# Distributed-Deep-Learning/ErasureHead

Hardware: AMD Instinct MI355X
Metric: wall-clock sec/iter + iters-to-loss-floor, logistic regression n_stragglers=2, 1/2/4/8 MI355X (lower is better)
Workload: dtype fp64

## Files before the change

### csrc/bindings.cpp

```cpp
#include <c10/hip/HIPStream.h>
#include <pybind11/stl.h>
#include <torch/extension.h>

#include <optional>
#include <stdexcept>
#include <string>
#include <tuple>
#include <vector>

#include "runtime/collector.h"

#include "kernels/grad_dense.h"
#include "kernels/launchers.h"

extern "C" const char eh_source_hash[];

namespace eh {
void bind_ipc(pybind11::module& m);
void bind_comm(pybind11::module& m);
void bind_engine(pybind11::module& m);
}

namespace {

// ... 29 lines not shown
       "part must hold [nslots*16*ld] partial sums (acc dtype)");
}

void grad_dense(int64_t dtype, int64_t loss, int64_t cpl, const Tensor& segs, const Tensor& tasks,
                const Tensor& beta, const Tensor& slab, const Tensor& slot_task_begin, const Tensor& part,
                const Tensor& G, int64_t ld, const eh::KernelChoice& choice) {
  need_cuda(segs, "segs");
  need_cuda(tasks, "tasks");
  need_cuda(beta, "beta");
  need_cuda(slab, "slab");
  need_cuda(slot_task_begin, "slot_task_begin");
  need_cuda(G, "G");
  const int64_t ntasks = tasks.size(0);
  const int64_t nslots = slot_task_begin.numel() - 1;
  need(tasks.dim() == 2 && tasks.size(1) == 5 && tasks.scalar_type() == at::kInt, "tasks must be int32 [ntasks, 5]");
  need(segs.scalar_type() == at::kByte && segs.numel() % 32 == 0, "segs must be packed uint8 [nseg*32]");
  need(slab.dim() == 2 && slab.size(0) >= ntasks && slab.size(1) == ld, "slab must be [>=ntasks, ld]");
  need(G.dim() == 2 && G.size(0) == nslots && G.size(1) == ld, "G must be [nslots, ld]");
  need(beta.numel() >= ld, "beta must have >= ld elements");
  need(ld % (dtype == 0 ? 2 : dtype == 1 ? 4 : 8) == 0, "ld must be a multiple of the 16-byte vector width");
  need(cpl <= 32 ? cpl * 64 >= ld
                   : ((cpl == 256 || cpl == 512) && cpl * (dtype == 0 ? 16 : 32) >= ld),
         "cpl (narrow: columns per lane, wide: block size) must cover ld");
  const int ac = dtype == 0 ? 0 : 1;
  need(acc_code(beta) == ac && acc_code(slab) == ac && acc_code(G) == ac, "beta/slab/G dtype mismatch");
  need_part(part, nslots, ld, ac);
  if (ntasks == 0) return;
  check(eh::grad_dense_launch((int)dtype, (int)loss, (int)cpl, segs.data_ptr(), tasks.data_ptr(), (int)ntasks,
                              beta.data_ptr(), slab.data_ptr(), slot_task_begin.data_ptr<int>(), (int)nslots,
                              part.data_ptr(), G.data_ptr(), (int)ld, stream_of(G), choice),
        "grad_dense");
}

void grad_dense_twopass(int64_t dtype, int64_t loss, const Tensor& segs, const Tensor& tasks,
                        const Tensor& beta, const Tensor& task_row_off, const Tensor& rbuf,
                        const Tensor& slab, const Tensor& slot_task_begin, const Tensor& part, const Tensor& G,
                        int64_t ld) {
  need_cuda(segs, "segs");
  need_cuda(tasks, "tasks");
  need_cuda(beta, "beta");
  need_cuda(task_row_off, "task_row_off");
  need_cuda(rbuf, "rbuf");
  need_cuda(slab, "slab");
  need_cuda(G, "G");
  const int64_t ntasks = tasks.size(0);
  const int64_t nslots = slot_task_begin.numel() - 1;
  need(slab.dim() == 2 && slab.size(0) >= ntasks && slab.size(1) == ld, "slab must be [>=ntasks, ld]");
  need(G.dim() == 2 && G.size(0) == nslots && G.size(1) == ld, "G must be [nslots, ld]");
  need(task_row_off.numel() >= ntasks, "task_row_off too small");
  need_part(part, nslots, ld, acc_code(G));
  need(rbuf.numel() >= 1 && acc_code(rbuf) == acc_code(G) && acc_code(beta) == acc_code(G), "rbuf/beta dtype");
  if (ntasks == 0) return;
  check(eh::grad_dense_twopass_launch((int)dtype, (int)loss, segs.data_ptr(), tasks.data_ptr(), (int)ntasks,
                                      beta.data_ptr(), task_row_off.data_ptr<int>(), rbuf.data_ptr(),
                                      slab.data_ptr(), slot_task_begin.data_ptr<int>(), (int)nslots,
                                      part.data_ptr(), G.data_ptr(), (int)ld, stream_of(G)),
        "grad_dense_twopass");
}

void encode_messages(const Tensor& Gb, const Tensor& ptr, const Tensor& idx, const Tensor& coef, const Tensor& G) {
  for (auto* p : {&Gb, &ptr, &idx, &coef, &G}) need_cuda(*p, "encode operand");
  need(ptr.scalar_type() == at::kInt && idx.scalar_type() == at::kInt, "ptr/idx must be int32");
  need(coef.scalar_type() == at::kDouble && coef.numel() == idx.numel(), "coef must be fp64, one per idx");
  const int ac = acc_code(G);
  need(acc_code(Gb) == ac && Gb.dim() == 2 && G.dim() == 2 && Gb.size(1) == G.size(1), "Gb/G mismatch");
  need(ptr.numel() == G.size(0) + 1, "ptr must have nslots + 1 entries");
// ... 102 lines not shown
}

void bind_kernel_choice(pybind11::module& m) {
  namespace py_ = pybind11;
  py_::class_<eh::KernelChoice>(m, "KernelChoice", "dense-gradient kernel selection (csrc/kernels/grad_dense.h)")
      .def(py_::init([](int kind, int replicas, int fold, int lane_epi, int pair, int wpr, int rows, int beta_lds) {
             return eh::KernelChoice{kind, replicas, fold, lane_epi, pair, wpr, rows, beta_lds};
           }),
           py_::arg("kind") = 0, py_::arg("replicas") = 1, py_::arg("fold") = 0, py_::arg("lane_epi") = 0,
           py_::arg("pair") = 0, py_::arg("wpr") = 0, py_::arg("rows") = 2, py_::arg("beta_lds") = 0)
      .def_readonly("kind", &eh::KernelChoice::kind)
      .def_readonly("replicas", &eh::KernelChoice::replicas)
      .def_readonly("fold", &eh::KernelChoice::fold)
      .def_readonly("lane_epi", &eh::KernelChoice::lane_epi)
      .def_readonly("pair", &eh::KernelChoice::pair)
      .def_readonly("wpr", &eh::KernelChoice::wpr)
      .def_readonly("rows", &eh::KernelChoice::rows)
      .def_readonly("beta_lds", &eh::KernelChoice::beta_lds);
}

}

PYBIND11_MODULE(TORCH_EXTENSION_NAME, m) {
  m.doc() = "ErasureHead MI355X native runtime: gfx950 HIP kernels + arrival collector + IPC mailbox";
  bind_kernel_choice(m);
  eh::bind_ipc(m);
  eh::bind_comm(m);
  eh::bind_engine(m);
  m.def("grad_dense", &grad_dense);
  m.def("set_mfma_stage_rows", &eh::set_mfma_stage_rows, "rows per LDS stage of the bf16 MFMA bundles: 32 (default) or 16");
  m.def("set_mfma_pack", &eh::set_mfma_pack, "bf16 MFMA bundles with R <= 4: terms packed into M (default) or one MFMA each");
  m.def("set_mfma_stream", &eh::set_mfma_stream, "packed bf16 MFMA bundles through the VGPR stream (A/B)");
  m.def("set_mfma_probe", &eh::set_mfma_probe, "timing probe of the MFMA bundles (not a gradient): 1 loads only, 2 compute only");
  m.def("set_slab_reduce_mode", &eh::set_slab_reduce_mode, "slab reduction form: 1 fused (default), 2 fused "
        "plain / two-stage puts, 0 two stages (same-box A/B)");
  m.def("slab_reduce_mode", &eh::slab_reduce_mode);
  m.def("set_release_form", &eh::set_release_form, pybind11::arg("strict"),
        "release form of every later put / signal / arbiter launch in this process (launchers.h)");
  m.def("strict_release", &eh::strict_release);
  m.def("_set_grad_stamps", [](uintptr_t p) { eh::set_grad_stamps(reinterpret_cast<void*>(p)); },
        "timeline probe of the one-wave bundles (tools/probes/bundle_stamps.py); 0 = off");
  m.def("grad_dense_twopass", &grad_dense_twopass);
  m.def("encode_messages", &encode_messages);
  m.def("combine_update", &combine_update);
  m.def("eval_gemm_loss", &eval_gemm_loss);
  m.def("eval_csr_loss", &eval_csr_loss);
  m.def("_mfma_probe", &mfma_probe);
  m.def("_tr_probe", &tr_probe);
  m.attr("MAX_MSGS") = eh::kMaxMsgs;
  m.attr("SOURCE_HASH") = std::string(eh_source_hash + sizeof("EH_SOURCE_HASH:") - 1);

  namespace py = pybind11;
  py::class_<eh::Arrival>(m, "Arrival")
      .def_readonly("worker", &eh::Arrival::worker)
      .def_readonly("part", &eh::Arrival::part)
      .def_readonly("round", &eh::Arrival::round)
      .def_readonly("t_rel", &eh::Arrival::t_rel)
      .def_readonly("probe", &eh::Arrival::probe)
      .def("__repr__", [](const eh::Arrival& a) {
        return "Arrival(worker=" + std::to_string(a.worker) + ", part=" + std::to_string(a.part) +
               ", round=" + std::to_string(a.round) + ", t_rel=" + std::to_string(a.t_rel) + ")";
      });
  py::class_<eh::Collector>(m, "Collector")
      .def(py::init<int, std::vector<int>, int>(), py::arg("n_workers"), py::arg("group_of"), py::arg("n_groups"))
      .def_static("now", &eh::Collector::now)
      .def("begin_round", &eh::Collector::begin_round)
      .def("set_tie_seed", &eh::Collector::set_tie_seed)
      .def("set_shards", &eh::Collector::set_shards)
      .def_property_readonly("tie_seed", &eh::Collector::tie_seed)
// ... 40 lines not shown
```

### csrc/kernels/grad_dense.hip

```cpp
#include <algorithm>
#include <cstdio>
#include <cstdlib>
#include <map>
#include <mutex>
#include <string>
#include <tuple>
#include <type_traits>

#include "common.h"
#include "grad_dense.h"
#include "launchers.h"
#include "lds_dma.h"

namespace eh {

template <typename T, typename A, int CPL, int LOSS, int ROWS, bool BL = false>
__global__ void __launch_bounds__(256)
grad_dense_fused(const Segment* __restrict__ segs, const Task* __restrict__ tasks,
                 const A* __restrict__ beta, A* __restrict__ slab, int ld, const int* __restrict__ gate) {
  constexpr int VN = Vec16<T>::N;
  constexpr int NV = CPL / VN;
  static_assert(CPL % VN == 0, "CPL must be a multiple of the vector width");
  if (gate_closed(gate)) return;

// ... 833 lines not shown
      const T* x1 = X + static_cast<long long>(two ? r + 1 : r) * ld;
      A a0[NV][VN], a1[NV][VN];
#pragma unroll
      for (int j = 0; j < NV; ++j) {
        const int c0 = (j * BS + tid) * VN;
        if (valid[j]) {
          Vec16<T>::template load<A, true>(x0 + c0, a0[j]);
          Vec16<T>::template load<A, true>(x1 + c0, a1[j]);
        } else {
#pragma unroll
          for (int v = 0; v < VN; ++v) { a0[j][v] = A(0); a1[j][v] = A(0); }
        }
      }
      pair(a0, a1, Y[r], two ? Y[r + 1] : A(0), two);
    }
  }
#pragma unroll
  for (int q = 0; q < R; ++q) {
    if (!act[q]) continue;
    A* out = slab + static_cast<long long>(tasks[blockIdx.x * R + q].slab) * ld;
#pragma unroll
    for (int j = 0; j < NV; ++j) {
      const int c0 = (j * BS + tid) * VN;
      if (valid[j]) {
#pragma unroll
        for (int v = 0; v < VN; ++v) out[c0 + v] = g[q][j][v];
      }
    }
  }
}

constexpr int kSplits = 16;
static int g_slab_mode = 1;
static long long* g_stamps = nullptr;

template <typename A>
__global__ void __launch_bounds__(256)
slab_reduce_partial(const A* __restrict__ slab, const int* __restrict__ slot_task_begin,
                    A* __restrict__ part, int ld, const int* __restrict__ gate) {
  __shared__ A red[4][kWave];
  if (gate_closed(gate)) return;
  const int slot = blockIdx.y, split = blockIdx.z;
  const int lane = threadIdx.x & 63, wid = threadIdx.x >> 6;
  const int c = blockIdx.x * kWave + lane;
  const int tb = slot_task_begin[slot], te = slot_task_begin[slot + 1];
  const int per = (te - tb + kSplits - 1) / kSplits;
  const int t0 = tb + split * per;
  const int t1 = min(te, t0 + per);
  A s = A(0);
  if (c < ld)
    for (int t = t0 + wid; t < t1; t += 4) s += slab[static_cast<long long>(t) * ld + c];
  red[wid][lane] = s;
  __syncthreads();
  if (wid == 0 && c < ld)
    part[(static_cast<long long>(slot) * kSplits + split) * ld + c] = (red[0][lane] + red[1][lane]) + (red[2][lane] + red[3][lane]);
}

template <typename A>
__global__ void __launch_bounds__(256)
slab_reduce_final(const A* __restrict__ part, A* __restrict__ G, int ld, const int* __restrict__ gate) {
  const int slot = blockIdx.y;
  const int c = blockIdx.x * blockDim.x + threadIdx.x;
  if (c >= ld || gate_closed(gate)) return;
  A s = A(0);
#pragma unroll
  for (int k = 0; k < kSplits; ++k) s += part[(static_cast<long long>(slot) * kSplits + k) * ld + c];
  G[static_cast<long long>(slot) * ld + c] = s;
}

template <typename A>
__device__ __forceinline__ A fused_split_sum(const A* __restrict__ slab, int t0, int t1, int ld, int c) {
  A acc[4] = {A(0), A(0), A(0), A(0)};
  int t = t0;
  for (; t + 8 <= t1; t += 8) {
    A v[8];
#pragma unroll
    for (int j = 0; j < 8; ++j) v[j] = slab[static_cast<long long>(t + j) * ld + c];
#pragma unroll
    for (int j = 0; j < 8; ++j) acc[j & 3] += v[j];
  }
  for (; t < t1; ++t) acc[(t - t0) & 3] += slab[static_cast<long long>(t) * ld + c];
  return (acc[0] + acc[1]) + (acc[2] + acc[3]);
}

template <typename A>
__device__ __forceinline__ A fused_slab_sum(const A* __restrict__ slab, const int* __restrict__ slot_task_begin,
                                            A (*red)[kWave], int slot, int ld, int c) {
  const int lane = threadIdx.x & 63, k = threadIdx.x >> 6;
  const int tb = slot_task_begin[slot], te = slot_task_begin[slot + 1];
  const int per = (te - tb + kSplits - 1) / kSplits;
  const int t0 = tb + k * per;
  const int t1 = min(te, t0 + per);
  red[k][lane] = c < ld && t0 < t1 ? fused_split_sum(slab, t0, t1, ld, c) : A(0);
  __syncthreads();
  A s = A(0);
  if (k == 0)
#pragma unroll
    for (int q = 0; q < kSplits; ++q) s += red[q][lane];
  return s;
}

template <typename A>
__global__ void __launch_bounds__(1024)
slab_reduce_fused(const A* __restrict__ slab, const int* __restrict__ slot_task_begin, A* __restrict__ G, int ld,
                  const int* __restrict__ gate) {
  __shared__ A red[kSplits][kWave];
  if (gate_closed(gate)) return;
  const int slot = blockIdx.y, c = blockIdx.x * kWave + (threadIdx.x & 63);
  const A s = fused_slab_sum(slab, slot_task_begin, red, slot, ld, c);
  if ((threadIdx.x >> 6) == 0 && c < ld) G[static_cast<long long>(slot) * ld + c] = s;
}

template <typename A>
__global__ void __launch_bounds__(1024)
slab_reduce_fused_put(const A* __restrict__ slab, const int* __restrict__ slot_task_begin, A* __restrict__ G, int ld,
                      PutDesc put) {
  __shared__ A red[kSplits][kWave];
  __shared__ int s_last, s_live;
// ... 122 lines not shown
      v0[k] = part[(static_cast<long long>(q0) * kSplits + k) * ld + c0];
      v1[k] = part[(static_cast<long long>(q1) * kSplits + k) * ld + c1];
    }
    A s0 = A(0), s1 = A(0);
#pragma unroll
    for (int k = 0; k < kSplits; ++k) {
      s0 += v0[k];
      s1 += v1[k];
    }
    G[e0] = s0;
    if (live) static_cast<A*>(put.dst)[e0] = s0;
    if (put.tag) atomicAdd(&tsum[q0], tag_term(elem_bits(s0), c0));
    if (two) {
      G[e1] = s1;
      if (live) static_cast<A*>(put.dst)[e1] = s1;
      if (put.tag) atomicAdd(&tsum[q1], tag_term(elem_bits(s1), c1));
    }
  }
  if (!live) return;
  if (put.tag) {
    __syncthreads();
    if (tid < nslots) put.tag[tid] = MsgTag{static_cast<unsigned int>(put.value), put.rank, tsum[tid]};
    if (put.corrupt && tid == 0) static_cast<unsigned char*>(put.dst)[1] ^= 0x10;
  }
  if (tid == 0) put_stamp(put);
  block_release_system(put.strict);
  if (tid == 0) {
    publish_u64(put.flag, put.value, put.strict);
    put_decide_next_gate(put);
  }
}

template <typename A>
__global__ void __launch_bounds__(1024)
slab_final_update(const A* __restrict__ part, A* __restrict__ G, int ld, int nslots, const LocalUpdate up) {
  extern __shared__ __attribute__((aligned(16))) unsigned char lu_raw[];
  A* gs = reinterpret_cast<A*>(lu_raw);
  const int lane = threadIdx.x & 63, wid = threadIdx.x >> 6;
  const int c = blockIdx.x * kWave + lane;
  if (up.stamp && blockIdx.x == 0 && threadIdx.x == 0) *up.stamp = wall_clock64();
  for (int q = wid; q < nslots; q += static_cast<int>(blockDim.x >> 6)) {
    A v = A(0);
    if (c < ld) {
#pragma unroll
      for (int k = 0; k < kSplits; ++k) v += part[(static_cast<long long>(q) * kSplits + k) * ld + c];
      G[static_cast<long long>(q) * ld + c] = v;
    }
    gs[q * kWave + lane] = v;
  }
  __syncthreads();
  if (wid != 0 || c >= ld) return;
  A* bw = static_cast<A*>(up.beta_w);
  if (c >= up.d) {
    if (bw) bw[c] = A(0);
    return;
  }
  double g = 0.0;
  for (int m = 0; m < up.nmsg; ++m) g = fma(up.coef[m], static_cast<double>(gs[up.slot[m] * kWave + lane]), g);
  const double b = up.beta[c];
  double nb;
  if (up.rule == 0) {
    nb = up.decay * b - up.gm * g;
  } else {
    const double yt = (1.0 - up.theta) * b + up.theta * up.u[c];
    nb = yt - up.gm * g - up.l2 * b;
    up.u[c] = b + (nb - b) * (1.0 / up.theta);
  }
  up.beta[c] = nb;
  if (up.hist) up.hist[c] = nb;
  if (bw) bw[c] = static_cast<A>(nb);
}

template <typename A>
static hipError_t slab_reduce_launch(const A* slab, const int* stb, A* part, A* G, int nslots, int ld,
                                     hipStream_t st, const PutDesc* put = nullptr, const int* gate = nullptr) {
  if (put && put->tag && (nslots > kMaxTagRows || !put->csum)) return hipErrorInvalidValue;
  if (put && put->gate != gate) return hipErrorInvalidValue;
  PutDesc pd{};
  if (put) {
    pd = *put;
    pd.strict = strict_release() ? 1 : 0;
    put = &pd;
  }
  const dim3 fgrid(ceil_div(ld, kWave), nslots);
  if (g_slab_mode != 0 && !put) {
    hipLaunchKernelGGL(slab_reduce_fused<A>, fgrid, dim3(1024), 0, st, slab, stb, G, ld, gate);
    return hipGetLastError();
  }
  if (g_slab_mode == 1 && put) {
    hipLaunchKernelGGL(slab_reduce_fused_put<A>, fgrid, dim3(1024), 0, st, slab, stb, G, ld, *put);
    return hipGetLastError();
  }
  hipLaunchKernelGGL(slab_reduce_partial<A>, dim3(ceil_div(ld, kWave), nslots, kSplits), dim3(256), 0, st,
                     slab, stb, part, ld, gate);
  if (put && nslots <= kPutOneSlots && static_cast<long long>(nslots) * ld <= kPutOneElems)
    hipLaunchKernelGGL(slab_reduce_final_put1<A>, dim3(1), dim3(1024), 0, st, part, G, ld, nslots, *put);
  else if (put)
    hipLaunchKernelGGL(slab_reduce_final_put<A>, dim3(ceil_div(ld, 256), nslots), dim3(256), 0, st, part, G, ld, *put);
  else
    hipLaunchKernelGGL(slab_reduce_final<A>, dim3(ceil_div(ld, 256), nslots), dim3(256), 0, st, part, G, ld, gate);
  return hipGetLastError();
}

// ... 30 lines not shown
template <typename T, typename A>
__global__ void __launch_bounds__(256)
xt_r_tiles(const Segment* __restrict__ segs, const Task* __restrict__ tasks,
           const int* __restrict__ task_row_off, const A* __restrict__ rbuf,
           A* __restrict__ slab, int ld, const int* __restrict__ gate) {
  constexpr int VN = Vec16<T>::N;
  if (gate_closed(gate)) return;
  const Task task = tasks[blockIdx.x];
  const Segment seg = segs[task.seg];
  const T* __restrict__ X = static_cast<const T*>(seg.X);
  const int off = task_row_off[blockIdx.x];
  const int c0 = (blockIdx.y * blockDim.x + threadIdx.x) * VN;
  if (c0 >= ld) return;
  A g[VN];
#pragma unroll
  for (int v = 0; v < VN; ++v) g[v] = A(0);
  for (int r = task.row_begin; r < task.row_end; ++r) {
    A a[VN];
    Vec16<T>::template load<A, true>(X + static_cast<long long>(r) * ld + c0, a);
    const A rr = rbuf[off + (r - task.row_begin)];
#pragma unroll
    for (int v = 0; v < VN; ++v) g[v] = fma(rr, a[v], g[v]);
  }
  A* out = slab + static_cast<long long>(task.slab) * ld + c0;
#pragma unroll
  for (int v = 0; v < VN; ++v) out[v] = g[v];
}

}

namespace eh {

void set_slab_reduce_mode(int mode) { g_slab_mode = mode; }
void set_grad_stamps(void* stamps) { g_stamps = static_cast<long long*>(stamps); }
int slab_reduce_mode() { return g_slab_mode; }

template <typename T, typename A, int LOSS>
static hipError_t launch_wide(int bs, int R, const Segment* segs, const Task* tasks, int ntasks, const A* beta,
                              A* slab, int ld, hipStream_t st, const int* gate) {
  constexpr int NV = Vec16<T>::N == 8 ? 4 : 8;
  if (R < 1 || R > 3 || ntasks % R) return hipErrorInvalidValue;
  const dim3 grid(ntasks / R);
  const bool half = static_cast<long long>(bs) * (NV / 2) * Vec16<T>::N >= ld;
  const bool quarter = NV >= 8 && static_cast<long long>(bs) * (NV / 4) * Vec16<T>::N >= ld;
#define EH_WIDE(NV_, BS_, R_)                                                                                     \
  hipLaunchKernelGGL((grad_dense_wide<T, A, NV_, BS_, LOSS, R_>), grid, dim3(BS_), 0, st, segs, tasks, beta, slab, ld, \
                     gate)
#define EH_WIDE_NV(BS_, R_)       \
  do {                            \
    if (quarter)                  \
      EH_WIDE(NV / 4, BS_, R_);   \
    else if (half)                \
      EH_WIDE(NV / 2, BS_, R_);   \
    else                          \
      EH_WIDE(NV, BS_, R_);       \
  } while (0)
  if (bs == 256 && R > 1 && !half) {
    if (R == 2)
      hipLaunchKernelGGL((grad_dense_wide<T, A, NV / 2, 512, LOSS, 2, true>), grid, dim3(512), 0, st, segs, tasks, beta,
                         slab, ld, gate);
    else
      hipLaunchKernelGGL((grad_dense_wide<T, A, NV / 2, 512, LOSS, 3, true>), grid, dim3(512), 0, st, segs, tasks, beta,
                         slab, ld, gate);
  } else if (bs == 256) {
    if (R == 1) EH_WIDE_NV(256, 1); else if (R == 2) EH_WIDE_NV(256, 2); else EH_WIDE_NV(256, 3);
  } else if (bs == 512 && R == 1) {
    EH_WIDE_NV(512, 1);
  } else {
// ... 109 lines not shown
      return hipErrorInvalidValue;
  }
#undef EH_IF
}

hipError_t grad_dense_launch(int dtype, int loss, int cpl, const void* segs, const void* tasks,
                             int ntasks, const void* beta, void* slab, const int* slot_task_begin,
                             int nslots, void* part, void* G, int ld, hipStream_t st, const KernelChoice& k,
                             const PutDesc* put, const int* gate) {
  const Segment* S = static_cast<const Segment*>(segs);
  const Task* Tk = static_cast<const Task*>(tasks);
  hipError_t e = hipSuccess;
  if (dtype == 0) {
    e = loss == kLogistic
            ? launch_fused_cpl<double, double, kLogistic>(cpl, S, Tk, ntasks, (const double*)beta, (double*)slab, ld, st, k, gate)
            : launch_fused_cpl<double, double, kLeastSquares>(cpl, S, Tk, ntasks, (const double*)beta, (double*)slab, ld, st, k, gate);
  } else if (dtype == 1) {
    e = loss == kLogistic
            ? launch_fused_cpl<float, float, kLogistic>(cpl, S, Tk, ntasks, (const float*)beta, (float*)slab, ld, st, k, gate)
            : launch_fused_cpl<float, float, kLeastSquares>(cpl, S, Tk, ntasks, (const float*)beta, (float*)slab, ld, st, k, gate);
  } else {
    e = loss == kLogistic
            ? launch_fused_cpl<bf16_t, float, kLogistic>(cpl, S, Tk, ntasks, (const float*)beta, (float*)slab, ld, st, k, gate)
            : launch_fused_cpl<bf16_t, float, kLeastSquares>(cpl, S, Tk, ntasks, (const float*)beta, (float*)slab, ld, st, k, gate);
  }
  if (e != hipSuccess) return e;
  if (dtype == 0) return slab_reduce_launch<double>((const double*)slab, slot_task_begin, (double*)part, (double*)G, nslots, ld, st, put, gate);
  return slab_reduce_launch<float>((const float*)slab, slot_task_begin, (float*)part, (float*)G, nslots, ld, st, put, gate);
}


hipError_t grad_dense_update_launch(int dtype, int loss, int cpl, const void* segs, const void* tasks, int ntasks,
                                    const void* beta, void* slab, const int* stb, int nslots, void* part, void* G,
                                    int ld, hipStream_t st, const KernelChoice& k, const LocalUpdate& up) {
  if (nslots < 1 || nslots > kMaxMsgs || up.nmsg < 0 || up.nmsg > kMaxMsgs || !up.beta) return hipErrorInvalidValue;
  for (int m = 0; m < up.nmsg; ++m)
    if (up.slot[m] < 0 || up.slot[m] >= nslots) return hipErrorInvalidValue;
  const Segment* S = static_cast<const Segment*>(segs);
  const Task* Tk = static_cast<const Task*>(tasks);
  hipError_t e;
  if (dtype == 0)
    e = loss == kLogistic ? launch_fused_cpl<double, double, kLogistic>(cpl, S, Tk, ntasks, (const double*)beta, (double*)slab, ld, st, k)
                          : launch_fused_cpl<double, double, kLeastSquares>(cpl, S, Tk, ntasks, (const double*)beta, (double*)slab, ld, st, k);
  else if (dtype == 1)
    e = loss == kLogistic ? launch_fused_cpl<float, float, kLogistic>(cpl, S, Tk, ntasks, (const float*)beta, (float*)slab, ld, st, k)
                          : launch_fused_cpl<float, float, kLeastSquares>(cpl, S, Tk, ntasks, (const float*)beta, (float*)slab, ld, st, k);
  else
    e = loss == kLogistic ? launch_fused_cpl<bf16_t, float, kLogistic>(cpl, S, Tk, ntasks, (const float*)beta, (float*)slab, ld, st, k)
                          : launch_fused_cpl<bf16_t, float, kLeastSquares>(cpl, S, Tk, ntasks, (const float*)beta, (float*)slab, ld, st, k);
  if (e != hipSuccess) return e;
  const dim3 pgrid(ceil_div(ld, kWave), nslots, kSplits);
  const size_t lds = static_cast<size_t>(nslots) * kWave * (dtype == 0 ? 8 : 4);
  auto go = [&](const void* kern) -> hipError_t {
    if (lds <= 60 * 1024) return hipSuccess;
    return hipFuncSetAttribute(kern, hipFuncAttributeMaxDynamicSharedMemorySize, static_cast<int>(lds));
  };
  if (dtype == 0) {
    hipLaunchKernelGGL(slab_reduce_partial<double>, pgrid, dim3(256), 0, st, (const double*)slab, stb, (double*)part, ld, nullptr);
    if ((e = go(reinterpret_cast<const void*>(slab_final_update<double>))) != hipSuccess) return e;
    hipLaunchKernelGGL(slab_final_update<double>, dim3(ceil_div(ld, kWave)), dim3(1024), lds, st, (const double*)part,
                       (double*)G, ld, nslots, up);
  } else {
    hipLaunchKernelGGL(slab_reduce_partial<float>, pgrid, dim3(256), 0, st, (const float*)slab, stb, (float*)part, ld, nullptr);
    if ((e = go(reinterpret_cast<const void*>(slab_final_update<float>))) != hipSuccess) return e;
    hipLaunchKernelGGL(slab_final_update<float>, dim3(ceil_div(ld, kWave)), dim3(1024), lds, st, (const float*)part,
                       (float*)G, ld, nslots, up);
  }
  return hipGetLastError();
}

hipError_t grad_dense_twopass_launch(int dtype, int loss, const void* segs, const void* tasks,
                                     int ntasks, const void* beta, const int* task_row_off,
                                     void* rbuf, void* slab, const int* slot_task_begin,
                                     int nslots, void* part, void* G, int ld, hipStream_t st, const int* gate) {
  const Segment* S = static_cast<const Segment*>(segs);
  const Task* Tk = static_cast<const Task*>(tasks);
  const dim3 block(256);
  if (dtype == 0) {
    if (loss == kLogistic)
      hipLaunchKernelGGL((rowdot_residual<double, double, kLogistic>), dim3(ntasks), block, 0, st, S, Tk, (const double*)beta, task_row_off, (double*)rbuf, ld, gate);
    else
      hipLaunchKernelGGL((rowdot_residual<double, double, kLeastSquares>), dim3(ntasks), block, 0, st, S, Tk, (const double*)beta, task_row_off, (double*)rbuf, ld, gate);
    hipLaunchKernelGGL((xt_r_tiles<double, double>), dim3(ntasks, ceil_div(ld, 256 * 2)), block, 0, st, S, Tk, task_row_off, (const double*)rbuf, (double*)slab, ld, gate);
// ... 21 lines not shown
```

### csrc/kernels/launchers.h

```cpp
#pragma once

#include <hip/hip_runtime.h>

#include <cstdlib>

#include "integrity.h"

namespace eh {

bool strict_release();
void set_release_form(bool strict);

constexpr long long kSlabSplits = 16;
inline long long slab_part_bytes(long long nslots, long long ld, long long acc_bytes) {
  return nslots * kSlabSplits * ld * acc_bytes;
}

struct PutDesc;
struct KernelChoice;
void set_slab_reduce_mode(int mode);
void set_mfma_stage_rows(int rows);
void set_mfma_probe(int mode);
void set_mfma_pack(bool on);
void set_mfma_stream(int mode);
void set_grad_stamps(void* stamps);
int slab_reduce_mode();
hipError_t grad_dense_launch(int dtype, int loss, int cpl, const void* segs, const void* tasks,
                             int ntasks, const void* beta, void* slab, const int* slot_task_begin,
                             int nslots, void* part, void* G, int ld, hipStream_t st, const KernelChoice& k,
                             const PutDesc* put = nullptr, const int* gate = nullptr);
hipError_t grad_dense_twopass_launch(int dtype, int loss, const void* segs, const void* tasks,
                                     int ntasks, const void* beta, const int* task_row_off,
                                     void* rbuf, void* slab, const int* slot_task_begin,
                                     int nslots, void* part, void* G, int ld, hipStream_t st,
                                     const int* gate = nullptr);
struct SparseArgs {
  int ell;
  int idx16;
  int m;
  long long nrows;
  const void* ell_idx;
  long long ell_ld;
  const int* lo;
  const long long* row_ptr;
  int csr_fixed;
  const int* col_idx;
  const void* vals;
  const void* y;
  void* u;
  int row16;
  const void* crow;
  const void* cvals;
  const int* col_ptr;
// ... 32 lines not shown

hipError_t encode_messages_launch(int dtype, const void* Gb, const int* ptr, const int* idx, const double* coef,
                                  void* G, int nslots, int ld, hipStream_t st, const int* gate = nullptr,
                                  const int* sub_begin = nullptr);

hipError_t eval_gemm_loss_launch(int x_dtype, int loss_kind, const void* X, long long ldx,
                                 long long n, int d, const void* y, const void* B, int ldb,
                                 int R, double* loss, void* P, hipStream_t st);

hipError_t eval_csr_loss_launch(int dtype, int loss_kind, const long long* row_ptr, const int* col, const void* vals,
                                long long n, const void* y, const void* Bt, int R, double* loss, void* P,
                                hipStream_t st);

constexpr int kMaxMsgs = 128;
struct CombineArgs {
  const void* msg[kMaxMsgs];
  double coef[kMaxMsgs];
  int nmsg;
};
struct LocalUpdate {
  int nmsg;
  int slot[kMaxMsgs];
  double coef[kMaxMsgs];
  double* beta;
  double* u;
  double* hist;
  void* beta_w;
  long long* stamp;
  int d, rule;
  double decay, gm, l2, theta;
};
hipError_t grad_dense_update_launch(int dtype, int loss, int cpl, const void* segs, const void* tasks, int ntasks,
                                    const void* beta, void* slab, const int* slot_task_begin, int nslots, void* part,
                                    void* G, int ld, hipStream_t st, const KernelChoice& k, const LocalUpdate& up);

hipError_t combine_update_launch(const CombineArgs& args, int msg_dtype, int w_dtype,
                                 double* beta, double* u, double* hist, void* beta_w,
                                 double* g_out, int d, int ld, double decay, double gm,
                                 double l2, double theta, int rule, hipStream_t st,
                                 long long* stamp = nullptr);
hipError_t stamp_launch(long long* out, hipStream_t st);

constexpr int kMaxPuts = 16;
struct PutDesc {
  const void* src;
  void* dst;
  long long bytes;
  unsigned long long* flag;
  unsigned long long value;
  unsigned int* counter;
  MsgTag* tag;
  unsigned long long* csum;
  int rows;
  int es;
  unsigned int rank;
  int corrupt;
  const int* abort;
  const int* gate;
  int* next_gate;
  const unsigned long long* beta_flag;
  unsigned long long stale_next;
  int strict;
  long long* stamp;
  long long* stamp_log;
};
#if defined(__HIPCC__)
__device__ __forceinline__ void put_stamp(const PutDesc& p) {
// ... 45 lines not shown
```

### csrc/runtime/engine.cpp

```cpp
#include <c10/hip/HIPStream.h>
#include <pybind11/stl.h>
#include <torch/extension.h>

#include <algorithm>
#include <array>
#include <chrono>
#include <cmath>
#include <cstdint>
#include <cstdio>
#include <cstring>
#include <map>
#include <memory>
#include <set>
#include <stdexcept>
#include <string>
#include <thread>
#include <tuple>
#include <vector>

#if defined(__x86_64__)
#include <immintrin.h>
#endif

#include <rocprofiler-sdk-roctx/roctx.h>
// ... 25 lines not shown
  }
  bool on;
};

namespace py = pybind11;
using at::Tensor;

void hcheck(hipError_t e, const char* what) {
  if (e != hipSuccess) throw std::runtime_error(std::string(what) + ": " + hipGetErrorString(e));
}

void need(bool ok, const std::string& msg) {
  if (!ok) throw std::invalid_argument(msg);
}

int acc_code(const Tensor& t) {
  if (t.scalar_type() == at::kDouble) return 0;
  if (t.scalar_type() == at::kFloat) return 1;
  throw std::invalid_argument("accumulator tensors must be float64 or float32");
}

void need_gpu(const Tensor& t, const char* name) {
  need(t.is_cuda() && t.is_contiguous(), std::string(name) + " must be a contiguous GPU tensor");
}

struct GradLauncher {
  int kind = 0;
  int dtype = 0, loss = 0, cpl = 0, ntasks = 0, nslots = 0, ld = 0;
  eh::KernelChoice choice{};
  const void* segs = nullptr;
  const void* tasks = nullptr;
  void* slab = nullptr;
  const int* stb = nullptr;
  void* part = nullptr;
  const int* task_row_off = nullptr;
  void* rbuf = nullptr;
  int acc = 0;
  eh::SparseArgs sa{};
  void* Gb = nullptr;
  const int* enc_ptr = nullptr;
  const int* enc_idx = nullptr;
  const double* enc_coef = nullptr;
  int enc_slots = 0;
  std::vector<Tensor> keep;

  hipError_t launch(const void* beta, void* G, hipStream_t st, const int* gate = nullptr) const {
    if (!Gb) return launch_raw(beta, G, st, gate);
    if (kind == 2 && sa.sub_begin) {
      eh::SparseArgs a = sa;
      a.Gb = Gb;
      a.encode_from_subs = 1;
      const hipError_t e = eh::grad_sparse_launch(acc, loss, a, beta, st, gate);
      if (e != hipSuccess) return e;
      return eh::encode_messages_launch(acc, sa.Gs, enc_ptr, enc_idx, enc_coef, G, enc_slots, ld, st, gate,
                                        sa.sub_begin);
    }
    const hipError_t e = launch_raw(beta, Gb, st, gate);
    if (e != hipSuccess) return e;
    return eh::encode_messages_launch(acc, Gb, enc_ptr, enc_idx, enc_coef, G, enc_slots, ld, st, gate);
  }

  bool can_fuse_put(int rows) const { return kind == 0 && !Gb && ntasks > 0 && nslots == rows; }
  bool can_fuse_update() const { return kind == 0 && !Gb && ntasks > 0; }
  hipError_t launch_update(const void* beta, void* G, const eh::LocalUpdate& up, hipStream_t st) const {
    return eh::grad_dense_update_launch(dtype, loss, cpl, segs, tasks, ntasks, beta, slab, stb, nslots, part, G, ld,
                                        st, choice, up);
  }
  hipError_t launch_put(const void* beta, void* G, const eh::PutDesc& put, hipStream_t st) const {
    return eh::grad_dense_launch(dtype, loss, cpl, segs, tasks, ntasks, beta, slab, stb, nslots, part, G, ld, st,
                                 choice, &put, put.gate);
  }

  hipError_t launch_raw(const void* beta, void* G, hipStream_t st, const int* gate = nullptr) const {
    switch (kind) {
      case 0:
        return ntasks ? eh::grad_dense_launch(dtype, loss, cpl, segs, tasks, ntasks, beta, slab, stb, nslots, part, G,
                                              ld, st, choice, nullptr, gate)
                      : hipSuccess;
      case 1:
        return ntasks ? eh::grad_dense_twopass_launch(dtype, loss, segs, tasks, ntasks, beta, task_row_off, rbuf, slab,
                                                      stb, nslots, part, G, ld, st, gate)
                      : hipSuccess;
      case 2: {
        eh::SparseArgs a = sa;
        a.Gb = G;
        if (!a.sub_begin) a.Gs = G;
        return eh::grad_sparse_launch(acc, loss, a, beta, st, gate);
      }
      default:
        return hipErrorInvalidValue;
    }
  }
};

std::shared_ptr<GradLauncher> make_dense(int64_t dtype, int64_t loss, int64_t cpl, const Tensor& segs,
                                         const Tensor& tasks, const Tensor& slab, const Tensor& stb,
                                         const Tensor& part, int64_t ld, std::optional<Tensor> task_row_off,
                                         std::optional<Tensor> rbuf, const eh::KernelChoice& choice) {
  for (auto* t : {&segs, &tasks, &slab, &stb, &part}) need_gpu(*t, "dense plan operand");
  need(tasks.dim() == 2 && tasks.size(1) == 5 && tasks.scalar_type() == at::kInt, "tasks must be int32 [n,5]");
  need(stb.scalar_type() == at::kInt, "slot_task_begin must be int32");
  auto g = std::make_shared<GradLauncher>();
  g->dtype = (int)dtype;
  g->loss = (int)loss;
  g->cpl = (int)cpl;
  g->choice = choice;
  g->ld = (int)ld;
  g->ntasks = (int)tasks.size(0);
  g->nslots = (int)stb.numel() - 1;
  need(part.numel() * part.element_size() >= eh::slab_part_bytes(g->nslots, ld, dtype == 0 ? 8 : 4),
       "part must hold the slab partial sums (grad.py DenseGradPlan)");
  g->segs = segs.data_ptr();
  g->tasks = tasks.data_ptr();
  g->slab = slab.data_ptr();
  g->stb = stb.data_ptr<int>();
  g->part = part.data_ptr();
  g->keep = {segs, tasks, slab, stb, part};
  g->acc = dtype == 0 ? 0 : 1;
  if (task_row_off) {
    need(rbuf.has_value(), "two-pass plan needs rbuf");
    need_gpu(*task_row_off, "task_row_off");
    need_gpu(*rbuf, "rbuf");
    g->kind = 1;
    g->task_row_off = task_row_off->data_ptr<int>();
    g->rbuf = rbuf->data_ptr();
    g->keep.push_back(*task_row_off);
    g->keep.push_back(*rbuf);
  } else {
    need(cpl <= 32 ? cpl * 64 >= ld
                   : ((cpl == 256 || cpl == 512) && cpl * (dtype == 0 ? 16 : 32) >= ld),
         "cpl (narrow: columns per lane, wide: block size) must cover ld");
    g->kind = 0;
  }
  return g;
}

std::shared_ptr<GradLauncher> make_sparse(int64_t loss, const Tensor& y, const Tensor& u, std::optional<Tensor> ell_idx,
                                          std::optional<Tensor> lo, std::optional<Tensor> row_ptr,
                                          std::optional<Tensor> col_idx, std::optional<Tensor> vals, const Tensor& crow,
                                          std::optional<Tensor> cvals, const Tensor& col_ptr, const Tensor& tiles,
                                          const Tensor& part_entry0, const Tensor& part_row0, const Tensor& part_nnz,
                                          const Tensor& head, const Tensor& tail, const Tensor& span,
                                          const Tensor& empty, int64_t nparts, int64_t d, int64_t ld,
                                          std::optional<Tensor> wg, int64_t u_lds, std::optional<Tensor> Gs,
                                          std::optional<Tensor> sub_begin, std::optional<Tensor> runs,
                                          std::optional<Tensor> tkeys, std::optional<Tensor> wspan,
                                          std::optional<Tensor> wspan_ptr, std::optional<Tensor> dst, int64_t csr_fixed) {
  for (auto* t : {&y, &u, &crow, &col_ptr, &tiles, &part_entry0, &part_row0, &part_nnz, &head, &tail, &span, &empty})
// ... 1894 lines not shown
```

Measured before the change: 0.001144.

## Fuse slab reduction, combine and local update into one batched launch

Replaces the two-launch slab reduce (per-slot partial kernel plus final combine/update kernel) on the local-update path with one kernel. Each block owns a column chunk, loops over slots in batches, reduces the split partial sums in LDS and applies the GD/AGD update from the combined gradient. Slot boundaries are copied to the host once at plan build and passed as a kernel-argument table, so the kernel needs no device lookups. The goal is to remove a launch and the partial-buffer round trip through global memory. The cost is fewer, heavier blocks with large LDS use, and a new tunable column-chunk width.

```diff
diff --git a/csrc/bindings.cpp b/csrc/bindings.cpp
--- a/csrc/bindings.cpp
+++ b/csrc/bindings.cpp
@@ -85,6 +85,66 @@
         "grad_dense");
 }
 
+void grad_dense_update(int64_t dtype, int64_t loss, int64_t cpl, const Tensor& segs, const Tensor& tasks,
+                       const Tensor& beta_w_in, const Tensor& slab, const Tensor& slot_task_begin, const Tensor& part,
+                       const Tensor& G, int64_t ld, const eh::KernelChoice& choice, const std::vector<int64_t>& slots,
+                       const std::vector<double>& coefs, const Tensor& beta, const Tensor& u, const OptT& hist,
+                       const OptT& beta_w, int64_t d, int64_t rule, double decay, double gm, double l2, double theta) {
+  for (auto* t : {&segs, &tasks, &beta_w_in, &slab, &slot_task_begin, &G, &beta, &u}) need_cuda(*t, "update operand");
+  const int64_t ntasks = tasks.size(0);
+  const int64_t nslots = slot_task_begin.numel() - 1;
+  need(tasks.dim() == 2 && tasks.size(1) == 5 && tasks.scalar_type() == at::kInt && ntasks > 0,
+       "tasks must be int32 [ntasks > 0, 5]");
+  need(segs.scalar_type() == at::kByte && segs.numel() % 32 == 0, "segs must be packed uint8 [nseg*32]");
+  need(slab.dim() == 2 && slab.size(0) >= ntasks && slab.size(1) == ld, "slab must be [>=ntasks, ld]");
+  need(nslots >= 1 && nslots <= eh::kMaxMsgs, "1 <= nslots <= MAX_MSGS");
+  need(G.dim() == 2 && G.size(0) == nslots && G.size(1) == ld, "G must be [nslots, ld]");
+  need(beta_w_in.numel() >= ld, "beta_w_in must have >= ld elements");
+  need(ld % (dtype == 0 ? 2 : dtype == 1 ? 4 : 8) == 0, "ld must be a multiple of the 16-byte vector width");
+  need(cpl <= 32 ? cpl * 64 >= ld : ((cpl == 256 || cpl == 512) && cpl * (dtype == 0 ? 16 : 32) >= ld),
+       "cpl (narrow: columns per lane, wide: block size) must cover ld");
+  const int ac = dtype == 0 ? 0 : 1;
+  need(acc_code(beta_w_in) == ac && acc_code(slab) == ac && acc_code(G) == ac, "beta_w_in/slab/G dtype mismatch");
+  need_part(part, nslots, ld, ac);
+  need(slot_task_begin.scalar_type() == at::kInt, "slot_task_begin must be int32");
+  const Tensor stb = slot_task_begin.cpu();
+  const int* sp = stb.data_ptr<int>();
+  need(sp[0] >= 0 && sp[nslots] <= slab.size(0), "slot_task_begin must address rows of slab");
+  for (int64_t q = 0; q < nslots; ++q) need(sp[q] <= sp[q + 1], "slot_task_begin must not decrease");
+  need(slots.size() == coefs.size() && static_cast<int>(slots.size()) <= eh::kMaxMsgs, "slots/coefs mismatch");
+  need(beta.scalar_type() == at::kDouble && u.scalar_type() == at::kDouble && beta.numel() == ld && u.numel() == ld,
+       "beta/u must be float64 [ld]");
+  need(d >= 0 && d <= ld && (rule == 0 || rule == 1), "d must be <= ld, rule 0 (GD) or 1 (AGD)");
+  eh::LocalUpdate up{};
+  up.nmsg = static_cast<int>(slots.size());
+  for (int m = 0; m < up.nmsg; ++m) {
+    need(slots[m] >= 0 && slots[m] < nslots, "slot out of range");
+    up.slot[m] = static_cast<int>(slots[m]);
+    up.coef[m] = coefs[m];
+  }
+  up.beta = beta.data_ptr<double>();
+  up.u = u.data_ptr<double>();
+  if (hist) {
+    need(hist->is_cuda() && hist->scalar_type() == at::kDouble && hist->numel() >= ld, "hist must be float64 [>= ld]");
+    up.hist = hist->data_ptr<double>();
+  }
+  if (beta_w) {
+    need_cuda(*beta_w, "beta_w");
+    need(beta_w->numel() == ld && acc_code(*beta_w) == ac, "beta_w must be [ld] in the message dtype");
+    up.beta_w = beta_w->data_ptr();
+  }
+  up.d = static_cast<int>(d);
+  up.rule = static_cast<int>(rule);
+  up.decay = decay;
+  up.gm = gm;
+  up.l2 = l2;
+  up.theta = theta;
+  check(eh::grad_dense_update_launch((int)dtype, (int)loss, (int)cpl, segs.data_ptr(), tasks.data_ptr(), (int)ntasks,
+                                     beta_w_in.data_ptr(), slab.data_ptr(), slot_task_begin.data_ptr<int>(),
+                                     (int)nslots, part.data_ptr(), G.data_ptr(), (int)ld, stream_of(G), choice, up, sp),
+        "grad_dense_update");
+}
+
 void grad_dense_twopass(int64_t dtype, int64_t loss, const Tensor& segs, const Tensor& tasks,
                         const Tensor& beta, const Tensor& task_row_off, const Tensor& rbuf,
                         const Tensor& slab, const Tensor& slot_task_begin, const Tensor& part, const Tensor& G,
@@ -253,9 +313,14 @@
   m.def("set_mfma_pack", &eh::set_mfma_pack, "bf16 MFMA bundles with R <= 4: terms packed into M (default) or one MFMA each");
   m.def("set_mfma_stream", &eh::set_mfma_stream, "packed bf16 MFMA bundles through the VGPR stream (A/B)");
   m.def("set_mfma_probe", &eh::set_mfma_probe, "timing probe of the MFMA bundles (not a gradient): 1 loads only, 2 compute only");
+  m.def("grad_dense_update", &grad_dense_update);
   m.def("set_slab_reduce_mode", &eh::set_slab_reduce_mode, "slab reduction form: 1 fused (default), 2 fused "
-        "plain / two-stage puts, 0 two stages (same-box A/B)");
+        "plain / two-stage puts, 0 two stages (same-box A/B); the local rounds' reduce + combine + update is one "
+        "launch under 1 and 2, two under 0");
   m.def("slab_reduce_mode", &eh::slab_reduce_mode);
+  m.def("set_slab_update_chunk", &eh::set_slab_update_chunk, "columns per block of the one-launch reduce + update: "
+        "16 (default), 32 or 64 (same-box sweep)");
+  m.def("slab_update_chunk", &eh::slab_update_chunk);
   m.def("set_release_form", &eh::set_release_form, pybind11::arg("strict"),
         "release form of every later put / signal / arbiter launch in this process (launchers.h)");
   m.def("strict_release", &eh::strict_release);
diff --git a/csrc/kernels/grad_dense.hip b/csrc/kernels/grad_dense.hip
--- a/csrc/kernels/grad_dense.hip
+++ b/csrc/kernels/grad_dense.hip
@@ -889,6 +889,7 @@
 
 constexpr int kSplits = 16;
 static int g_slab_mode = 1;
+static int g_slab_chunk = 16;
 static long long* g_stamps = nullptr;
 
 template <typename A>
@@ -941,6 +942,21 @@
 }
 
 template <typename A>
+__device__ __forceinline__ void split_rows_add(A (&acc)[4], const A* __restrict__ slab, int t, int t1, int ld, int c) {
+  for (; t + 8 <= t1; t += 8) {
+    A v[8];
+#pragma unroll
+    for (int j = 0; j < 8; ++j) v[j] = slab[static_cast<long long>(t + j) * ld + c];
+#pragma unroll
+    for (int j = 0; j < 8; ++j) acc[j & 3] += v[j];
+  }
+  for (; t < t1; t += 4)
+#pragma unroll
+    for (int j = 0; j < 4; ++j)
+      if (t + j < t1) acc[j] += slab[static_cast<long long>(t + j) * ld + c];
+}
+
+template <typename A>
 __device__ __forceinline__ A fused_slab_sum(const A* __restrict__ slab, const int* __restrict__ slot_task_begin,
                                             A (*red)[kWave], int slot, int ld, int c) {
   const int lane = threadIdx.x & 63, k = threadIdx.x >> 6;
@@ -1129,6 +1145,29 @@
 }
 
 template <typename A>
+__device__ __forceinline__ void local_update_col(const LocalUpdate& up, const A* gs, int stride, int c, double b,
+                                                 double uc) {
+  A* bw = static_cast<A*>(up.beta_w);
+  if (c >= up.d) {
+    if (bw) bw[c] = A(0);
+    return;
+  }
+  double g = 0.0;
+  for (int m = 0; m < up.nmsg; ++m) g = fma(up.coef[m], static_cast<double>(gs[up.slot[m] * stride]), g);
+  double nb;
+  if (up.rule == 0) {
+    nb = fma(up.decay, b, -(up.gm * g));
+  } else {
+    const double yt = fma(1.0 - up.theta, b, up.theta * uc);
+    nb = fma(-up.l2, b, fma(-up.gm, g, yt));
+    up.u[c] = fma(1.0 / up.theta, nb - b, b);
+  }
+  up.beta[c] = nb;
+  if (up.hist) up.hist[c] = nb;
+  if (bw) bw[c] = static_cast<A>(nb);
+}
+
+template <typename A>
 __global__ void __launch_bounds__(1024)
 slab_final_update(const A* __restrict__ part, A* __restrict__ G, int ld, int nslots, const LocalUpdate up) {
   extern __shared__ __attribute__((aligned(16))) unsigned char lu_raw[];
@@ -1147,25 +1186,101 @@
   }
   __syncthreads();
   if (wid != 0 || c >= ld) return;
-  A* bw = static_cast<A*>(up.beta_w);
-  if (c >= up.d) {
-    if (bw) bw[c] = A(0);
-    return;
-  }
-  double g = 0.0;
-  for (int m = 0; m < up.nmsg; ++m) g = fma(up.coef[m], static_cast<double>(gs[up.slot[m] * kWave + lane]), g);
-  const double b = up.beta[c];
-  double nb;
-  if (up.rule == 0) {
-    nb = up.decay * b - up.gm * g;
-  } else {
-    const double yt = (1.0 - up.theta) * b + up.theta * up.u[c];
-    nb = yt - up.gm * g - up.l2 * b;
-    up.u[c] = b + (nb - b) * (1.0 / up.theta);
-  }
-  up.beta[c] = nb;
-  if (up.hist) up.hist[c] = nb;
-  if (bw) bw[c] = static_cast<A>(nb);
+  local_update_col(up, gs + lane, kWave, c, up.beta[c], up.rule == 0 ? 0.0 : up.u[c]);
+}
+
+constexpr int kSlabBatch = 6;
+struct SlotTable {
+  int begin[kMaxMsgs + 1];
+  int maxper;
+};
+
+template <typename A, int SB, int NR>
+__device__ __forceinline__ void first_rows(A (&acc)[SB][4], const A* __restrict__ slab, const int (&t0)[SB],
+                                           const int (&n)[SB], int tlast, int ld, int cl, bool colok) {
+  A v[SB][NR];
+#pragma unroll
+  for (int s = 0; s < SB; ++s)
+#pragma unroll
+    for (int j = 0; j < NR; ++j) v[s][j] = slab[static_cast<long long>(min(t0[s] + j, tlast)) * ld + cl];
+#pragma unroll
+  for (int s = 0; s < SB; ++s)
+#pragma unroll
+    for (int j = 0; j < 4; ++j) acc[s][j] = A(0);
+#pragma unroll
+  for (int s = 0; s < SB; ++s)
+#pragma unroll
+    for (int j = 0; j < NR; ++j) acc[s][j] += colok && j < n[s] ? v[s][j] : A(0);
+}
+
+template <typename A, int CW>
+__global__ void __launch_bounds__(1024)
+slab_reduce_update(const A* __restrict__ slab, A* __restrict__ G, int ld, int nslots, const SlotTable tab,
+                   const LocalUpdate up) {
+  constexpr int NSUB = kWave / CW;
+  constexpr int SB = kSlabBatch;
+  constexpr int SBT = SB * NSUB;
+  static_assert(SBT * CW <= 1024, "one thread per (slot, column) of a batch");
+  extern __shared__ __attribute__((aligned(16))) unsigned char ru_raw[];
+  A* red = reinterpret_cast<A*>(ru_raw);
+  A* gs = red + SBT * kSplits * CW;
+  const int tid = threadIdx.x, lane = tid & 63, k = tid >> 6;
+  const int sub = lane / CW, cc = lane % CW;
+  const int c = blockIdx.x * CW + cc;
+  const bool colok = c < ld;
+  const int cl = min(c, ld - 1);
+  const bool upd = tid < CW && colok;
+  double b = 0.0, uc = 0.0;
+  if (upd) {
+    b = up.beta[c];
+    if (up.rule != 0) uc = up.u[c];
+  }
+  const int maxper = tab.maxper;
+  const int tlast = max(tab.begin[nslots] - 1, 0);
+  for (int qb = 0; qb < nslots; qb += SBT) {
+    int t0[SB], n[SB];
+#pragma unroll
+    for (int s = 0; s < SB; ++s) {
+      int tb = 0, te = 0;
+#pragma unroll
+      for (int u = 0; u < NSUB; ++u) {
+        const int q = qb + s * NSUB + u, qc = min(q, nslots - 1);
+        const int b0 = tab.begin[qc], e0 = tab.begin[qc + 1];
+        const int mine = -static_cast<int>(sub == u), real = -static_cast<int>(q < nslots);
+        tb |= b0 & mine;
+        te |= (b0 + ((e0 - b0) & real)) & mine;
+      }
+      const int per = (te - tb + kSplits - 1) / kSplits;
+      t0[s] = tb + k * per;
+      n[s] = max(min(te, t0[s] + per) - t0[s], 0);
+    }
+    A acc[SB][4];
+    if (maxper <= 1) first_rows<A, SB, 1>(acc, slab, t0, n, tlast, ld, cl, colok);
+    else if (maxper == 2) first_rows<A, SB, 2>(acc, slab, t0, n, tlast, ld, cl, colok);
+    else if (maxper == 3) first_rows<A, SB, 3>(acc, slab, t0, n, tlast, ld, cl, colok);
+    else first_rows<A, SB, 4>(acc, slab, t0, n, tlast, ld, cl, colok);
+    if (maxper > 4) {
+#pragma unroll
+      for (int s = 0; s < SB; ++s)
+        if (colok && n[s] > 4) split_rows_add(acc[s], slab, t0[s] + 4, t0[s] + n[s], ld, c);
+    }
+#pragma unroll
+    for (int s = 0; s < SB; ++s)
+      red[((s * NSUB + sub) * kSplits + k) * CW + cc] = (acc[s][0] + acc[s][1]) + (acc[s][2] + acc[s][3]);
+    __syncthreads();
+    if (tid < SBT * CW && qb + tid / CW < nslots) {
+      const int sl = tid / CW, c2 = tid % CW, q = qb + sl, gc = blockIdx.x * CW + c2;
+      A v = A(0);
+#pragma unroll
+      for (int j = 0; j < kSplits; ++j) v += red[(sl * kSplits + j) * CW + c2];
+      if (gc < ld) G[static_cast<long long>(q) * ld + gc] = v;
+      gs[q * CW + c2] = v;
+    }
+    __syncthreads();
+  }
+  if (up.stamp && blockIdx.x == 0 && tid == 0) *up.stamp = wall_clock64();
+  if (!upd) return;
+  local_update_col(up, gs + tid, CW, c, b, uc);
 }
 
 template <typename A>
@@ -1262,8 +1377,25 @@
 namespace eh {
 
 void set_slab_reduce_mode(int mode) { g_slab_mode = mode; }
+void set_slab_update_chunk(int cols) { g_slab_chunk = cols == 64 || cols == 32 ? cols : 16; }
+int slab_update_chunk() { return g_slab_chunk; }
 void set_grad_stamps(void* stamps) { g_stamps = static_cast<long long*>(stamps); }
 int slab_reduce_mode() { return g_slab_mode; }
+
+template <typename A, int CW>
+static hipError_t slab_reduce_update_launch(const A* slab, const SlotTable& tab, A* G, int ld, int nslots,
+                                            const LocalUpdate& up, hipStream_t st) {
+  constexpr int SBT = kSlabBatch * (kWave / CW);
+  const size_t lds = (static_cast<size_t>(SBT) * kSplits * CW + static_cast<size_t>(nslots) * CW) * sizeof(A);
+  const void* kern = reinterpret_cast<const void*>(slab_reduce_update<A, CW>);
+  if (lds > 60 * 1024) {
+    const hipError_t e = hipFuncSetAttribute(kern, hipFuncAttributeMaxDynamicSharedMemorySize, static_cast<int>(lds));
+    if (e != hipSuccess) return e;
+  }
+  hipLaunchKernelGGL((slab_reduce_update<A, CW>), dim3(ceil_div(ld, CW)), dim3(1024), lds, st, slab, G, ld, nslots, tab,
+                     up);
+  return hipGetLastError();
+}
 
 template <typename T, typename A, int LOSS>
 static hipError_t launch_wide(int bs, int R, const Segment* segs, const Task* tasks, int ntasks, const A* beta,
@@ -1439,7 +1571,8 @@
 
 hipError_t grad_dense_update_launch(int dtype, int loss, int cpl, const void* segs, const void* tasks, int ntasks,
                                     const void* beta, void* slab, const int* stb, int nslots, void* part, void* G,
-                                    int ld, hipStream_t st, const KernelChoice& k, const LocalUpdate& up) {
+                                    int ld, hipStream_t st, const KernelChoice& k, const LocalUpdate& up,
+                                    const int* stb_host) {
   if (nslots < 1 || nslots > kMaxMsgs || up.nmsg < 0 || up.nmsg > kMaxMsgs || !up.beta) return hipErrorInvalidValue;
   for (int m = 0; m < up.nmsg; ++m)
     if (up.slot[m] < 0 || up.slot[m] >= nslots) return hipErrorInvalidValue;
@@ -1456,6 +1589,27 @@
     e = loss == kLogistic ? launch_fused_cpl<bf16_t, float, kLogistic>(cpl, S, Tk, ntasks, (const float*)beta, (float*)slab, ld, st, k)
                           : launch_fused_cpl<bf16_t, float, kLeastSquares>(cpl, S, Tk, ntasks, (const float*)beta, (float*)slab, ld, st, k);
   if (e != hipSuccess) return e;
+  if (g_slab_mode != 0) {
+    if (!stb_host) return hipErrorInvalidValue;
+    SlotTable tab{};
+    for (int q = 0; q <= nslots; ++q) tab.begin[q] = stb_host[q];
+    for (int q = 0; q < nslots; ++q) {
+      if (stb_host[q] < 0 || stb_host[q + 1] < stb_host[q]) return hipErrorInvalidValue;
+      tab.maxper = std::max(tab.maxper, (stb_host[q + 1] - stb_host[q] + kSplits - 1) / kSplits);
+    }
+    const bool f64 = dtype == 0;
+    switch (g_slab_chunk) {
+      case 16:
+        return f64 ? slab_reduce_update_launch<double, 16>((const double*)slab, tab, (double*)G, ld, nslots, up, st)
+                   : slab_reduce_update_launch<float, 16>((const float*)slab, tab, (float*)G, ld, nslots, up, st);
+      case 32:
+        return f64 ? slab_reduce_update_launch<double, 32>((const double*)slab, tab, (double*)G, ld, nslots, up, st)
+                   : slab_reduce_update_launch<float, 32>((const float*)slab, tab, (float*)G, ld, nslots, up, st);
+      default:
+        return f64 ? slab_reduce_update_launch<double, 64>((const double*)slab, tab, (double*)G, ld, nslots, up, st)
+                   : slab_reduce_update_launch<float, 64>((const float*)slab, tab, (float*)G, ld, nslots, up, st);
+    }
+  }
   const dim3 pgrid(ceil_div(ld, kWave), nslots, kSplits);
   const size_t lds = static_cast<size_t>(nslots) * kWave * (dtype == 0 ? 8 : 4);
   auto go = [&](const void* kern) -> hipError_t {
diff --git a/csrc/kernels/launchers.h b/csrc/kernels/launchers.h
--- a/csrc/kernels/launchers.h
+++ b/csrc/kernels/launchers.h
@@ -19,6 +19,8 @@
 struct PutDesc;
 struct KernelChoice;
 void set_slab_reduce_mode(int mode);
+void set_slab_update_chunk(int cols);
+int slab_update_chunk();
 void set_mfma_stage_rows(int rows);
 void set_mfma_probe(int mode);
 void set_mfma_pack(bool on);
@@ -117,7 +119,8 @@
 };
 hipError_t grad_dense_update_launch(int dtype, int loss, int cpl, const void* segs, const void* tasks, int ntasks,
                                     const void* beta, void* slab, const int* slot_task_begin, int nslots, void* part,
-                                    void* G, int ld, hipStream_t st, const KernelChoice& k, const LocalUpdate& up);
+                                    void* G, int ld, hipStream_t st, const KernelChoice& k, const LocalUpdate& up,
+                                    const int* slot_task_begin_host);
 
 hipError_t combine_update_launch(const CombineArgs& args, int msg_dtype, int w_dtype,
                                  double* beta, double* u, double* hist, void* beta_w,
diff --git a/csrc/runtime/engine.cpp b/csrc/runtime/engine.cpp
--- a/csrc/runtime/engine.cpp
+++ b/csrc/runtime/engine.cpp
@@ -81,6 +81,7 @@
   const void* tasks = nullptr;
   void* slab = nullptr;
   const int* stb = nullptr;
+  std::vector<int> stb_host;
   void* part = nullptr;
   const int* task_row_off = nullptr;
   void* rbuf = nullptr;
@@ -113,7 +114,7 @@
   bool can_fuse_update() const { return kind == 0 && !Gb && ntasks > 0; }
   hipError_t launch_update(const void* beta, void* G, const eh::LocalUpdate& up, hipStream_t st) const {
     return eh::grad_dense_update_launch(dtype, loss, cpl, segs, tasks, ntasks, beta, slab, stb, nslots, part, G, ld,
-                                        st, choice, up);
+                                        st, choice, up, stb_host.data());
   }
   hipError_t launch_put(const void* beta, void* G, const eh::PutDesc& put, hipStream_t st) const {
     return eh::grad_dense_launch(dtype, loss, cpl, segs, tasks, ntasks, beta, slab, stb, nslots, part, G, ld, st,
@@ -163,6 +164,10 @@
   g->tasks = tasks.data_ptr();
   g->slab = slab.data_ptr();
   g->stb = stb.data_ptr<int>();
+  {
+    const Tensor h = stb.cpu().contiguous();
+    g->stb_host.assign(h.data_ptr<int>(), h.data_ptr<int>() + h.numel());
+  }
   g->part = part.data_ptr();
   g->keep = {segs, tasks, slab, stb, part};
   g->acc = dtype == 0 ? 0 : 1;
```

Measured after the change: 0.001140, median of 6. No clear change (-0.4%).
